# ratt-ru/pfb-imaging

Measured on AMD Instinct MI355X. Metric: Mvis/s gridded+degridded in exact Hessian applies (8192^2 grid, 1e7 vis/band), higher is better.
Workload: dtype f64

## Files before the change

### pfb-imaging_amd/csrc/gridder.hip

```cpp
#include <hip/hip_runtime.h>
#include <rocfft/rocfft.h>

#include <hipcub/hipcub.hpp>

#include <algorithm>
#include <chrono>
#include <cmath>
#include <cstdlib>
#include <string>
#include <cstring>
#include <memory>
#include <vector>

#include "common.hpp"
#include "devcg.hpp"
#include "eskernel.hpp"
#include "gridder_kernels_mp.hpp"
#include "gridder_wd_api.hpp"
#include "rowfft_api.hpp"
#include "vismap.hpp"

namespace pfbhip {

constexpr double SPEED_OF_LIGHT = 299792458.0;
// ... 568 lines not shown
        for (int q = 0; q < 3; ++q) ga.wshare[q] = wshare[q];
        return ga;
    }
    template <int W>
    size_t lds_bytes_mp() const
    {
        constexpr int D = kernel_poly_degree_c(W);
        static_assert(kernel_poly_degree_c(W) == kernel_poly_degree(W), "degree mismatch");
        return (size_t(2) * size_t(kp_max) * tile_rows(W) * tile_stride(W) + size_t(W) * (D + 1)) * sizeof(double);
    }
    template <int W>
    static constexpr size_t lds_bytes_mp_max()
    {
        constexpr int D = kernel_poly_degree_c(W);
        return (size_t(2) * KP_MAX * tile_rows(W) * tile_stride(W) + size_t(W) * (D + 1)) * sizeof(double);
    }
    template <int W, int KP>
    void launch_grid_mp_wk(const GroupArgs &ga, const double2 *sval)
    {
        allow_dynamic_lds(reinterpret_cast<const void *>(&k_grid_mp<W, KP>), int(lds_bytes_mp_max<W>()));
        hipLaunchKernelGGL((k_grid_mp<W, KP>), dim3(ga.a.nwork), dim3(MP_THREADS), lds_bytes_mp<W>(), stream, ga, sval,
                           grid_cur);
    }
    template <int W, int KP>
    size_t lds_bytes_blk() const
    {
        return (size_t(2) * KP * blk_tile_rows(W) * blk_stride(W, KP) + blk_fixed_doubles(W, blk_threads(kp_max) / 64)) * sizeof(double);
    }
    template <int W, int KP, int BC>
    void launch_grid_blk_wkb(const GroupArgs &ga, const double2 *sval)
    {
        allow_dynamic_lds(reinterpret_cast<const void *>(&k_grid_blk<W, KP, BC>), 160 * 1024);
        const size_t lds = lds_bytes_blk<W, KP>();
        PFB_REQUIRE(lds <= size_t(160) * 1024, "block scatter needs %zu bytes of LDS", lds);
        hipLaunchKernelGGL((k_grid_blk<W, KP, BC>), dim3(ga.a.nwork), dim3(blk_threads(kp_max)), lds, stream, ga, sval, grid_cur);
    }
    template <int W, int KP>
    void launch_grid_blk_wk(const GroupArgs &ga, const double2 *sval)
    {
        if constexpr (W == 14 || W == 15) {
            if (wd_bc == 2) return launch_grid_blk_wkb<W, KP, 2>(ga, sval);
        }
        launch_grid_blk_wkb<W, KP, 4>(ga, sval);
    }
    bool scatter_blk = true;
    bool scatter_rec = false, pval_ready = false, want_pval = false;
    WdArgs wd{};
    int wd_bc = 4;
    DevBuf<double> d_dtab;
    DevBuf<double2> d_cw;
    bool wd_small = false;
    int pval_per_vis() const { return info.wmode == 2 ? wd.K : kp_max; }
    bool pval_from_gather = false;
    DevBuf<VisRec> d_rec;
    bool gather_rw = false;
    DevBuf<double> d_kw;
    float wshare[3] = {1.3f / 3, 1.f / 3, 0.7f / 3};
    DevBuf<double2> d_pval;
    template <int W, int KP, int BC>
    void launch_grid_rec_wkb(const GroupArgs &ga)
    {
        allow_dynamic_lds(reinterpret_cast<const void *>(&k_grid_rec<W, KP, BC>), 160 * 1024);
        const size_t lds = lds_bytes_blk<W, KP>();
        PFB_REQUIRE(lds <= size_t(160) * 1024, "record scatter needs %zu bytes of LDS", lds);
        hipLaunchKernelGGL((k_grid_rec<W, KP, BC>), dim3(ga.a.nwork), dim3(blk_threads(kp_max)), lds, stream, ga, d_rec.p, d_pval.p,
                           grid_cur);
    }
    template <int W, int KP>
    void launch_grid_rec_wk(const GroupArgs &ga)
    {
        if constexpr (W == 14 || W == 15) {
            if (wd_bc == 2) return launch_grid_rec_wkb<W, KP, 2>(ga);
        }
        launch_grid_rec_wkb<W, KP, 4>(ga);
    }
    template <int W>
    void launch_grid_mp_w(int plane0, int kp, const double2 *sval)
    {
        GroupArgs ga = group_args(plane0, kp);
        if (ga.a.nwork == 0) return;
        if (scatter_blk) {
            const size_t grp = work_off.size() > 1 ? size_t(plane0 / kp_max) : 0;
            if (scatter_rec && !pval_ready) {
                timer.begin(5);
                if (info.wmode == 2)
                    wd_launch_plane_values(wd.K, info.nactive, d_cw.p, sval, d_pval.p, stream);
                else if (prm.do_wgridding && info.wmode == 0)
                    hipLaunchKernelGGL((k_plane_values_es<W>), dim3(ga.a.nwork), dim3(256), 0, stream, ga, sval, d_pval.p);
                else
                    hipLaunchKernelGGL((k_plane_values<W>), dim3(uint32_t(ceil_div(info.nactive, 256))), dim3(256), 0, stream, ga,
                                       info.nactive, sval, d_pval.p);
                timer.end();
            }
            for (int col = 0; col < 4; ++col) {
                ga.a.work = d_work_col.p + col_off[grp * 4 + size_t(col)];
                ga.a.nwork = uint32_t(col_cnt[grp * 4 + size_t(col)]);
                if (ga.a.nwork == 0) continue;
                timer.begin(0);
                if (info.wmode == 2) {
                    wd_launch_grid(ga, wd, d_rec.p, d_pval.p, grid_cur, stream);
                    timer.end();
                    continue;
                }
                if (scatter_rec) {
                    switch (kp) {
                        case 1: launch_grid_rec_wk<W, 1>(ga); break;
                        case 2: launch_grid_rec_wk<W, 2>(ga); break;
                        case 3: launch_grid_rec_wk<W, 3>(ga); break;
                        default: launch_grid_rec_wk<W, 4>(ga); break;
                    }
                    timer.end();
                    continue;
                }
                switch (kp) {
                    case 1: launch_grid_blk_wk<W, 1>(ga, sval); break;
                    case 2: launch_grid_blk_wk<W, 2>(ga, sval); break;
                    case 3: launch_grid_blk_wk<W, 3>(ga, sval); break;
                    default: launch_grid_blk_wk<W, 4>(ga, sval); break;
                }
                timer.end();
            }
            return;
        }
        timer.begin(0);
        switch (kp) {
            case 1: launch_grid_mp_wk<W, 1>(ga, sval); break;
            case 2: launch_grid_mp_wk<W, 2>(ga, sval); break;
            case 3: launch_grid_mp_wk<W, 3>(ga, sval); break;
            default: launch_grid_mp_wk<W, 4>(ga, sval); break;
        }
        timer.end();
    }
    template <int W, int KP>
    void launch_degrid_mp_wk(const GroupArgs &ga, double2 *sacc)
    {
        allow_dynamic_lds(reinterpret_cast<const void *>(&k_degrid_mp<W, KP>), int(lds_bytes_mp_max<W>()));
        hipLaunchKernelGGL((k_degrid_mp<W, KP>), dim3(ga.a.nwork), dim3(MP_THREADS), lds_bytes_mp<W>(), stream, ga,
                           grid_cur, sacc, want_pval ? d_swgt.p : nullptr, want_pval ? d_pval.p : nullptr);
    }
    template <int W, int KP>
    void launch_degrid_rw_wk(const GroupArgs &ga, double2 *sacc)
    {
        allow_dynamic_lds(reinterpret_cast<const void *>(&k_degrid_rw<W, KP>), 160 * 1024);
        const size_t lds = size_t(KP) * RW_LS * RW_LS * sizeof(double2);
        hipLaunchKernelGGL((k_degrid_rw<W, KP>), dim3(ga.a.nwork), dim3(MP_THREADS), lds, stream, ga, d_rec.p, d_kw.p, grid_cur,
                           sacc, want_pval ? d_swgt.p : nullptr, want_pval ? d_pval.p : nullptr);
    }
    template <int W>
    void launch_degrid_mp_w(int plane0, int kp, double2 *sacc)
    {
        GroupArgs ga = group_args(plane0, kp);
        if (ga.a.nwork == 0) return;
        if (info.wmode == 2) {
// ... 136 lines not shown
    }

    FusedGeom fgeom;
    const FusedGeom &fused_geom() const { return fgeom; }
    std::vector<FusedPlanes> plane_groups;
    DevBuf<double2> d_tau;
    FusedPlanes fused_planes(int p0, int kp) const
    {
        const size_t grp = size_t(p0 / kp_max);
        if (grp < plane_groups.size() && plane_groups[grp].kp == kp) return plane_groups[grp];
        FusedPlanes fp;
        fp.kp = kp;
        for (int k = 0; k < FUSED_MAXPLANES; ++k) fp.w[k] = k < kp ? wplanes[size_t(p0 + k)] : 0.0;
        return fp;
    }

    void finalize(const double *beam, double scale, double eta, const double *x, double *out)
    {
        const int64_t npix = int64_t(prm.nx) * prm.ny;
        timer.begin(5);
        hipLaunchKernelGGL(k_finalize_img, dim3(uint32_t(ceil_div(npix, 256))), dim3(256), 0, stream, d_accT.p, d_corr.p, beam, scale,
                           eta, x, npix, out);
        PFB_HIP(hipGetLastError());
        timer.end();
    }

    void prepare_degrid_input(const double *x, const double *beam)
    {
        const int64_t npix = int64_t(prm.nx) * prm.ny;
        timer.begin(5);
        hipLaunchKernelGGL(k_prepare_img, dim3(uint32_t(ceil_div(npix, 256))), dim3(256), 0, stream, x, d_corr.p, beam, npix,
                           d_accT.p);
        PFB_HIP(hipGetLastError());
        timer.end();
    }

    void prepare_and_degrid(const double *x, const double *beam, double2 *sacc)
    {
        if (side_clear_pending && info.nplanes == 1) side_clear();
        if (fused && info.nactive != 0 && info.nwork != 0 && fused_pad_takes_prep(rowfft_u, fgeom)) {
            FusedPrep p;
            p.x = x;
            p.corr = d_corr.p;
            p.beam = beam;
            degrid_all_planes(sacc, &p);
        } else {
            prepare_degrid_input(x, beam);
            degrid_all_planes(sacc);
        }
    }

    void degrid_all_planes(double2 *sacc, const FusedPrep *prep = nullptr)
    {
        if (!want_pval) PFB_HIP(hipMemsetAsync(sacc, 0, size_t(std::max<int64_t>(info.nactive, 1)) * sizeof(double2), stream));
        if (info.nactive == 0 || info.nwork == 0) return;
        for (int p0 = 0; p0 < info.nplanes; p0 += kp_max) {
            const int kp = int(std::min<int64_t>(kp_max, info.nplanes - p0));
            if (fused) {
                timer.begin(7);
                fused_pad_fft(rowfft_u, fused_geom(), d_occ.p, d_accT.p, prep != nullptr ? *prep : FusedPrep{},
                              fused_planes(p0, kp), prm.do_wgridding, d_gridB.p, bstride, stream);
                timer.end();
            }
            if (tfft) {
                timer.begin(2);
                rowfft_b2a(rowfft_v.pl, d_gridB.p, grid_cur, d_rowmap.p, int(occ_rows), geom.bpitch, int(prm.ny), size_t(geom.apitch),
                           fgeom.tpitch, kp, plane_stride, bstride, d_colruns.p, stream);
                timer.end();
            }
            for (int k = 0; k < kp && !tfft; ++k) {
                const int p = p0 + k;
                if (!fused) {
                    timer.begin(3);
                    hipLaunchKernelGGL(k_pad_screen_T, dim3(uint32_t(ceil_div(info.nu, 256)), uint32_t(prm.ny)),
                                       dim3(256), 0, stream, geom, fgeom, d_accT.p, prm.do_wgridding, wplanes[size_t(p)],
                                       d_gridB.p);
                    PFB_HIP(hipGetLastError());
                    timer.end();
                    fft_rows_B(true);
                }
                timer.begin(3);
                hipLaunchKernelGGL(k_b2a, tgrid(info.nu, info.nv), dim3(TP, TRANSPOSE_ROWS), 0, stream, geom, d_occ.p,
                                   d_gridB.p + (fused ? size_t(k) * bstride : 0), grid_cur + size_t(k) * plane_stride);
                PFB_HIP(hipGetLastError());
                timer.end();
                fft_rows_A(true, k);
            }
            if (side_clear_pending) side_clear();
            timer.begin(1);
            PFB_W_DISPATCH(launch_degrid_mp_w, p0, kp, sacc);
            PFB_HIP(hipGetLastError());
            timer.end();
        }
    }

    DevBuf<float> d_stage32;
    void upload_f32(const float *host, size_t n, double *dst)
    {
        d_stage32.ensure(n);
        PFB_HIP(hipMemcpyAsync(d_stage32.p, host, n * sizeof(float), hipMemcpyHostToDevice, stream));
        hipLaunchKernelGGL(k_widen_f32, dim3(uint32_t(ceil_div(int64_t(n), 256))), dim3(256), 0, stream, int64_t(n), d_stage32.p, dst);
        PFB_HIP(hipGetLastError());
    }
    void download_f32(const double *src, size_t n, float *host)
    {
        d_stage32.ensure(n);
        hipLaunchKernelGGL(k_narrow_f64, dim3(uint32_t(ceil_div(int64_t(n), 256))), dim3(256), 0, stream, int64_t(n), src, d_stage32.p);
        PFB_HIP(hipGetLastError());
        PFB_HIP(hipMemcpyAsync(host, d_stage32.p, n * sizeof(float), hipMemcpyDeviceToHost, stream));
    }
    void upload_vis_wgt_sp(const float *vis_host, const float *wgt_host)
    {
        if (vis_host) {
            d_vis.ensure(size_t(nvis));
            upload_f32(vis_host, size_t(nvis) * 2, reinterpret_cast<double *>(d_vis.p));
        }
        if (wgt_host) {
            d_wgt.ensure(size_t(nvis));
            upload_f32(wgt_host, size_t(nvis), d_wgt.p);
        }
    }
    void upload_vis_wgt(const double *vis_host, const double *wgt_host)
    {
        if (vis_host) {
            d_vis.ensure(size_t(nvis));
            PFB_HIP(hipMemcpyAsync(d_vis.p, vis_host, size_t(nvis) * sizeof(double2), hipMemcpyHostToDevice, stream));
        }
        if (wgt_host) {
            d_wgt.ensure(size_t(nvis));
            PFB_HIP(hipMemcpyAsync(d_wgt.p, wgt_host, size_t(nvis) * sizeof(double), hipMemcpyHostToDevice, stream));
        }
    }
};

namespace pfbhip {

static inline dim3 blocks1d(int64_t n, int t = 256) { return dim3(uint32_t(std::max<int64_t>(ceil_div(n, t), 1))); }

static double fft2d_seconds(int64_t nu, int64_t nv)
{
    static const struct { int64_t n; double ms; } meas[] = {
// ... 49 lines not shown
    if (!(smax >= 0.0 && smax < 1.0)) return HUGE_VAL;
    double tq[WD_MAX_K], M[WD_MAX_K][WD_MAX_K];
    wd_interp_nodes(K, smax, nshift, tq, M);
    double worst = 0.0;
    for (int iw = 0; iw <= WD_ERR_NW; ++iw) {
        const double dwv = whalf * (double(iw) / (0.5 * WD_ERR_NW) - 1.0);
        double cr[WD_MAX_K], ci[WD_MAX_K];
        for (int k = 0; k < K; ++k) {
            cr[k] = ci[k] = 0.0;
            for (int q = 0; q < K; ++q) {
                cr[k] += M[k][q] * std::cos(2.0 * pi_const * dwv * tq[q]);
                ci[k] -= M[k][q] * std::sin(2.0 * pi_const * dwv * tq[q]);
            }
        }
        for (int is = 0; is <= WD_ERR_NS; ++is) {
            const double x = double(is) / double(WD_ERR_NS), sv = x * smax;
            const double tt = -sv / (1.0 + std::sqrt(1.0 - sv)) + nshift;
            double ar = 0.0, ai = 0.0, xp = 1.0;
            for (int k = 0; k < K; ++k) {
                ar += cr[k] * xp;
                ai += ci[k] * xp;
                xp *= x;
            }
            const double e = std::hypot(ar - std::cos(2.0 * pi_const * dwv * tt), ai + std::sin(2.0 * pi_const * dwv * tt));
            if (!std::isfinite(e)) return HUGE_VAL;
            worst = std::max(worst, e);
        }
    }
    return worst;
}

static double wd_smax(const pfbhip_gridder_params &p)
{
    const double xe = double(p.nx / 2) * p.pixsize_x, ye = double(p.ny / 2) * p.pixsize_y;
    return xe * xe + ye * ye;
}

static double w_interp_budget(const pfbhip_gridder_params &p, double nmin)
{
    return 2.0 * p.epsilon / 3.0 * (p.divide_by_n ? std::max(0.25, std::min(1.0, nmin)) : 1.0);
}

enum class ScatterForce { Auto, Walk, Block, Rec, RecEs };
struct PlanSwitches {
    ScatterForce scatter = ScatterForce::Auto;
    bool wmode2 = true;
    bool wd_block4 = false;
    int wd_colours = -1;
    bool rowfft = true;
    bool fused_fft = true;
    int fused_doubled = -1;
    bool sepscreen = true;
    bool tfft = true;
};

static PlanSwitches read_plan_switches()
{
    PlanSwitches sw;
    auto first = [](const char *name) -> int {
        const char *e = std::getenv(name);
        return e == nullptr ? -1 : e[0];
    };
    if (const char *e = std::getenv("PFBHIP_SCATTER")) {
        const std::string v(e);
        if (v == "auto") sw.scatter = ScatterForce::Auto;
        else if (v == "walk") sw.scatter = ScatterForce::Walk;
        else if (v == "block") sw.scatter = ScatterForce::Block;
        else if (v == "rec") sw.scatter = ScatterForce::Rec;
        else if (v == "rec_es") sw.scatter = ScatterForce::RecEs;
        else PFB_REQUIRE(false, "PFBHIP_SCATTER=%s: expected auto, walk, block, rec or rec_es", e);
    }
    sw.wmode2 = first("PFBHIP_WMODE2") != '0';
    sw.wd_block4 = first("PFBHIP_WD_BLOCK") == '4';
    const int wc = first("PFBHIP_WD_COLOURS");
    sw.wd_colours = wc == '0' ? 0 : (wc == '1' ? 1 : -1);
    sw.rowfft = first("PFBHIP_ROWFFT") != '0';
    sw.fused_fft = first("PFBHIP_FUSED_FFT") != '0';
    const int fd = first("PFBHIP_FUSED_DOUBLED");
    sw.fused_doubled = fd < 0 ? -1 : (fd == '1' ? 1 : 0);
    sw.sepscreen = first("PFBHIP_SEPSCREEN") != '0';
    sw.tfft = first("PFBHIP_TFFT") != '0';
    return sw;
}

static void choose_kernel(pfbhip_gridder *g, const PlanSwitches &sw, double wlo, double whi, double tmax, double nmin)
{
    const auto &prm = g->prm;
    size_t nrows = 0;
    const KernelRow *tab = kernel_table(&nrows);
    const double eps1 = 0.8 / 1.25 * prm.epsilon / (prm.do_wgridding ? 3.0 : 2.0) *
                        ((prm.do_wgridding && prm.divide_by_n) ? std::max(0.25, std::min(1.0, nmin)) : 1.0);
    const double eps_w = 0.5 * w_interp_budget(prm, nmin);
    const double nvis = double(g->nvis);
    const bool wgrid = prm.do_wgridding && tmax > 0.0;
    const double pi = 3.14159265358979323846;
    double best_cost = 1e300;
    const KernelRow *best = nullptr;
    int64_t bnu = 0, bnv = 0, bnpl = 1;
    double bdw = 1.0;
    int bmode = 0, bnder = 0;
    const bool wd_allowed = sw.wmode2 && g->info.lshift == 0.0 && g->info.mshift == 0.0 &&
                            (sw.scatter == ScatterForce::Auto || sw.scatter == ScatterForce::Rec);
    const double wd_omega = 2.0 * pi * 0.5 * (whi - wlo) * tmax;
    int wd_K = 0;
    if (wgrid && wd_allowed) {
        const int K0 = poly_planes_needed(wd_omega, 2.0 * eps_w);
        for (int K = K0; K >= 2 && K <= WD_MAX_K; ++K)
            if (wd_interp_error(K, wd_smax(prm), 0.5 * (whi - wlo), g->info.nshift) <= 2.0 * eps_w) {
                wd_K = K;
                break;
            }
    }
    for (size_t i = 0; i < nrows; ++i) {
        const KernelRow &r = tab[i];
        if (prm.force_W > 0) {
            if (r.W != prm.force_W || std::fabs(r.sigma - prm.force_sigma) > 1e-9) continue;
        } else {
            if (r.sigma < prm.sigma_min - 1e-9 || r.sigma > prm.sigma_max + 1e-9 || r.eps_sup > eps1) continue;
        }
        double rounding_es = 0.0, rounding_poly = 0.0;
        int64_t cand_u[2] = {grid_size(prm.nx, r.sigma), rowfft_size_at_least(double(prm.nx) * r.sigma)};
        int64_t cand_v[2] = {grid_size(prm.ny, r.sigma), rowfft_size_at_least(double(prm.ny) * r.sigma)};
        for (int cand = 0; cand < 2; ++cand) {
            const int64_t nu = cand_u[cand], nv = cand_v[cand];
            if (nu <= 0 || nv <= 0) continue;
            if (cand == 1 && (nu == cand_u[0] && nv == cand_v[0])) continue;
            if (cand == 1 && prm.force_W <= 0 &&
                (double(nu) > prm.sigma_max * double(prm.nx) || double(nv) > prm.sigma_max * double(prm.ny)))
                continue;
            if (prm.force_W <= 0) {
                const KernelFT ft(r.W, r.beta);
                const double f0 = ft(0.0);
                double amp = (f0 / ft(0.5 * double(prm.nx) / double(nu))) * (f0 / ft(0.5 * double(prm.ny) / double(nv)));
                if (wgrid) amp = std::max(amp, amp * f0 / ft(0.5 / r.sigma));
// ... 449 lines not shown
            wd_interp_nodes(K, smax, info.nshift, wa.tq, wa.M);
            g->d_cw.alloc((size_t(info.nactive) + REC_PAD) * size_t(K));
            wa.cw = g->d_cw.p;
            wd_launch_coeffs(wa, info.nactive, g->d_pw.p, g->d_cw.p, st);
            const double worst = wd_interp_error(K, smax, info.whalf, info.nshift), bound = w_interp_budget(prm, 1.0 + nm1min);
            if (prm.verbosity > 0) fprintf(stderr, "[pfbhip] one-plane w-scheme: K = %d, interpolation error %.3g\n", K, worst);
            PFB_REQUIRE(worst <= bound, "one-plane w-scheme: interpolation error %g exceeds its share %g of epsilon %g", worst, bound,
                        prm.epsilon);
        }
        PFB_HIP(hipStreamSynchronize(st));
    }

    const int64_t npix = prm.nx * prm.ny;
    KernelFT ft(info.W, info.beta);
    std::vector<double> cfu = ft.correction_1d(prm.nx, info.nu);
    std::vector<double> cfv = (prm.ny == prm.nx && info.nv == info.nu) ? cfu : ft.correction_1d(prm.ny, info.nv);
    g->d_cfu.alloc(cfu.size());
    g->d_cfv.alloc(cfv.size());
    PFB_HIP(hipMemcpyAsync(g->d_cfu.p, cfu.data(), cfu.size() * sizeof(double), hipMemcpyHostToDevice, st));
    PFB_HIP(hipMemcpyAsync(g->d_cfv.p, cfv.data(), cfv.size() * sizeof(double), hipMemcpyHostToDevice, st));
    std::vector<double> cheb{1.0};
    double zmax = 1.0;
    const bool use_psiw = prm.do_wgridding && tmax > 0.0 && info.wmode == 0;
    if (use_psiw) {
        zmax = tmax * info.dw * (1.0 + 1e-12);
        cheb = ft.inverse_cheb(zmax);
    }
    g->d_cheb.alloc(cheb.size());
    PFB_HIP(hipMemcpyAsync(g->d_cheb.p, cheb.data(), cheb.size() * sizeof(double), hipMemcpyHostToDevice, st));
    g->d_corr.alloc(size_t(npix));
    hipLaunchKernelGGL(k_corr_image, blocks1d(npix), dim3(256), 0, st, g->geom, g->d_cfu.p, g->d_cfv.p, g->d_cheb.p,
                       int(cheb.size()), info.dw, zmax, prm.do_wgridding ? 1 : 0, use_psiw ? 1 : 0, prm.divide_by_n,
                       g->d_corr.p);
    PFB_HIP(hipGetLastError());

    lap("kernel table + correction");
    {
        RowFFTPlan probe;
        const bool own_v = sw.rowfft && rowfft_make_plan(info.nv, &probe);
        g->geom.apitch = int(info.nv) + (own_v ? 8 : 0);
    }
    g->plane_stride = size_t(info.nu) * size_t(g->geom.apitch);
    g->d_grid.alloc(g->plane_stride * size_t(g->kp_max));
    g->grid_cur = g->d_grid.p;
    {
        g->async_clear = info.nplanes <= g->kp_max && info.nactive > 0 && g->d_grid.bytes() <= (size_t(40) << 30);
        if (g->async_clear) {
            g->d_grid2.alloc(g->plane_stride * size_t(g->kp_max));
            PFB_HIP(hipStreamCreateWithFlags(&g->clear_stream, hipStreamNonBlocking));
            PFB_HIP(hipEventCreateWithFlags(&g->ev_clear, hipEventDisableTiming));
            PFB_HIP(hipEventCreateWithFlags(&g->ev_start, hipEventDisableTiming));
            PFB_HIP(hipMemsetAsync(g->d_grid2.p, 0, g->d_grid2.bytes(), st));
        }
    }
    lap("uv-plane buffers");
    g->d_img.alloc(size_t(npix));
    g->d_sval.alloc(size_t(std::max<int64_t>(info.nactive, 1)));
    g->d_sacc.alloc(size_t(std::max<int64_t>(info.nactive, 1)));

    const bool own_rows = sw.rowfft;
    const bool want_fused = sw.fused_fft;
    if (own_rows || want_fused) (void)g->rowfft_u.init(info.nu);
    const bool fuse_doubled = sw.fused_doubled >= 0 ? sw.fused_doubled == 1 : fused_doubled_stashes(g->rowfft_u);
    {
        FusedGeom &fg = g->fgeom;
        fg.nx = int(prm.nx);
        fg.ny = int(prm.ny);
        fg.nu = int(info.nu);
        fg.px = prm.pixsize_x;
        fg.py = prm.pixsize_y;
        fg.lshift = info.lshift;
        fg.mshift = info.mshift;
        fg.nshift = info.nshift;
        if (prm.do_wgridding) fused_geom_fit(fg);
        if (prm.verbosity > 0) fprintf(stderr, "[pfbhip] w-screen: n-1 polynomial with %d coefficients\n", fg.npoly);
    }
    g->fused = want_fused && g->rowfft_u.ok && (!g->rowfft_u.pl.doubled || fuse_doubled) &&
               (!prm.do_wgridding || g->fgeom.npoly > 0);
    if (!own_rows && !g->fused) g->rowfft_u.release();
    if (own_rows) (void)g->rowfft_v.init(info.nv);
    g->plane_groups.clear();
    g->d_tau.release();
    if (g->fused) {
        bool any_sep = false;
        for (int p0 = 0; p0 < info.nplanes; p0 += g->kp_max) {
            FusedPlanes fp;
            fp.kp = int(std::min<int64_t>(g->kp_max, info.nplanes - p0));
            for (int k = 0; k < FUSED_MAXPLANES; ++k) fp.w[k] = k < fp.kp ? g->wplanes[size_t(p0 + k)] : 0.0;
            if (prm.do_wgridding && !g->rowfft_u.pl.doubled) fused_planes_fit(g->fgeom, fp);
            if (fp.nsc == 0 && sw.sepscreen && prm.do_wgridding) fused_planes_fit(g->fgeom, fp, true);
            any_sep = any_sep || fp.sep != 0;
            g->plane_groups.push_back(fp);
        }
        if (any_sep) {
            g->d_tau.alloc(size_t(info.nplanes) * size_t(prm.nx));
            DevBuf<double> d_w(size_t(info.nplanes));
            PFB_HIP(hipMemcpyAsync(d_w.p, g->wplanes.data(), size_t(info.nplanes) * sizeof(double), hipMemcpyHostToDevice, st));
            fused_screen_table(g->fgeom, d_w.p, int(info.nplanes), g->d_tau.p, st);
            PFB_HIP(hipStreamSynchronize(st));
            for (size_t grp = 0; grp < g->plane_groups.size(); ++grp)
                g->plane_groups[grp].tau = g->d_tau.p + grp * size_t(g->kp_max) * size_t(prm.nx);
        }
        if (prm.verbosity > 0 && !g->plane_groups.empty()) {
            int n_sc = 0, n_sep = 0, nsc_max = 0;
            for (const FusedPlanes &fp : g->plane_groups) {
                n_sc += fp.nsc > 0 && !fp.sep;
// ... 332 lines not shown
                for (int64_t a = a0; a < std::min(a0 + 32, pu); ++a)
                    for (int64_t b = b0; b < std::min(b0 + 32, pv); ++b) out[b * pu + a] = tmp[a * int64_t(g->geom.apitch) + b];
    });
}

int pfbhip_gridder_dirty2vis(pfbhip_gridder *g, const double *dirty_host, const double *wgt_host, double *vis_host)
{
    return guarded([&] {
        PFB_REQUIRE(g && dirty_host && (vis_host || g->nvis == 0), "NULL argument");
        hipStream_t st = g->stream;
        const int64_t npix = g->prm.nx * g->prm.ny;
        PFB_HIP(hipMemcpyAsync(g->d_img.p, dirty_host, size_t(npix) * sizeof(double), hipMemcpyHostToDevice, st));
        g->upload_vis_wgt(nullptr, wgt_host);
        g->prepare_and_degrid(g->d_img.p, nullptr, g->d_sacc.p);
        if (g->nvis) {
            g->d_vis.ensure(size_t(g->nvis));
            PFB_HIP(hipMemsetAsync(g->d_vis.p, 0, size_t(g->nvis) * sizeof(double2), st));
            if (g->info.nactive)
                hipLaunchKernelGGL(k_permute_out, blocks1d(g->info.nactive), dim3(256), 0, st, g->map, g->d_src.p,
                                   g->info.nactive, g->d_sacc.p, wgt_host ? g->d_wgt.p : nullptr, int(g->shifting),
                                   g->info.lshift, g->info.mshift, g->info.nshift, g->d_vis.p);
            PFB_HIP(hipGetLastError());
            PFB_HIP(hipMemcpyAsync(vis_host, g->d_vis.p, size_t(g->nvis) * sizeof(double2), hipMemcpyDeviceToHost, st));
        }
        PFB_HIP(hipStreamSynchronize(st));
    });
}

int pfbhip_gridder_set_weights(pfbhip_gridder *g, const double *wgt_host)
{
    return guarded([&] {
        PFB_REQUIRE(g, "NULL handle");
        hipStream_t st = g->stream;
        g->upload_vis_wgt(nullptr, wgt_host);
        g->d_swgt.ensure(size_t(std::max<int64_t>(g->info.nactive, 1)));
        if (g->info.nactive)
            hipLaunchKernelGGL(k_gather_f64, blocks1d(g->info.nactive), dim3(256), 0, st, g->d_src.p, g->info.nactive,
                               wgt_host ? g->d_wgt.p : nullptr, g->d_swgt.p);
        PFB_HIP(hipGetLastError());
        PFB_HIP(hipStreamSynchronize(st));
        g->weights_bound = true;
    });
}

static void apply_op(pfbhip_gridder *g, const double *x_dev, const double *beam_dev, const double *beam_out_dev, double scale,
                     double eta, const double *addend_dev, double *out_dev)
{
    PFB_REQUIRE(g->weights_bound, "call pfbhip_gridder_set_weights before the Hessian");
    hipStream_t st = g->stream;
    const int64_t npix = g->prm.nx * g->prm.ny;
    const bool side = g->async_clear && g->info.nwork > 0;
    g->side_clear_pending = side;
    g->side_clear_done = false;
    g->want_pval = g->pval_from_gather && g->info.nwork > 0;
    struct ClearFlags {
        pfbhip_gridder *g;
        ~ClearFlags() { g->want_pval = g->pval_ready = false; }
    } clear_flags{g};
    g->prepare_and_degrid(x_dev, beam_dev, g->d_sacc.p);
    g->side_clear_pending = false;
    if (g->want_pval) {
        g->want_pval = false;
        g->pval_ready = true;
    } else {
        g->timer.begin(5);
        if (g->info.nactive)
            hipLaunchKernelGGL(k_scale_sorted, blocks1d(g->info.nactive), dim3(256), 0, st, g->info.nactive, g->d_sacc.p,
                               g->d_swgt.p, g->d_sval.p);
        PFB_HIP(hipGetLastError());
        g->timer.end();
    }
    if (g->side_clear_done) {
        PFB_HIP(hipStreamWaitEvent(st, g->ev_clear, 0));
        g->grid_cur = g->d_grid2.p;
        g->planes_cleared = true;
    }
    struct Restore {
        pfbhip_gridder *g;
        ~Restore()
        {
            g->grid_cur = g->d_grid.p;
            g->planes_cleared = false;
        }
    } restore{g};
    g->grid_and_finalize(g->d_sval.p, beam_out_dev, scale, eta, (eta != 0.0) ? addend_dev : nullptr, out_dev);
    (void)npix;
}

static void hessian_dev_impl(pfbhip_gridder *g, const double *x_dev, const double *beam_dev, double eta, double wsum,
                             double *out_dev)
{
    apply_op(g, x_dev, beam_dev, beam_dev, wsum > 0.0 ? 1.0 / wsum : 1.0, eta, eta != 0.0 ? x_dev : nullptr, out_dev);
}

int pfbhip_gridder_residual_dev(pfbhip_gridder *g, const double *model_dev, const double *beam_dev, const double *acc_dev,
                                double *out_dev)
{
    return guarded([&] {
        PFB_REQUIRE(g && model_dev && acc_dev && out_dev, "NULL argument");
        PFB_REQUIRE(model_dev != out_dev, "the residual cannot overwrite the model image");
        apply_op(g, model_dev, beam_dev, nullptr, -1.0, 1.0, acc_dev, out_dev);
        PFB_HIP(hipStreamSynchronize(g->stream));
    });
}

int pfbhip_gridder_hessian_dev(pfbhip_gridder *g, const double *x_dev, const double *beam_dev, double eta, double wsum,
                               double *out_dev)
{
    return guarded([&] {
        PFB_REQUIRE(g && x_dev && out_dev, "NULL argument");
        PFB_REQUIRE(x_dev != out_dev, "in-place Hessian is not supported");
        hessian_dev_impl(g, x_dev, beam_dev, eta, wsum, out_dev);
        PFB_HIP(hipStreamSynchronize(g->stream));
    });
// ... 210 lines not shown
```

### pfb-imaging_amd/csrc/gridder_kernels_wd.hpp

```cpp
#pragma once
#include "gridder_wd_api.hpp"

namespace pfbhip {

__host__ __device__ constexpr int wd_binom(int n, int r)
{
    return r == 0 || r == n ? 1 : (n == 2 ? 2 : (n == 3 ? 3 : 1));
}

__global__ void k_wd_coeffs(WdArgs wa, int64_t nactive, const double *__restrict__ pw, double2 *__restrict__ cw)
{
    const int64_t j = blockIdx.x * int64_t(blockDim.x) + threadIdx.x;
    if (j >= nactive + REC_PAD) return;
    double er[WD_MAX_K], ei[WD_MAX_K];
    const double dw = j < nactive ? pw[j] * wa.whalf : 0.0;
    for (int q = 0; q < wa.K; ++q) {
        double ph = dw * wa.tq[q];
        ph -= rint(ph);
        double s, c;
        sincospi(-2.0 * ph, &s, &c);
        er[q] = c;
        ei[q] = s;
    }
    for (int k = 0; k < wa.K; ++k) {
// ... 287 lines not shown
                for (int r = 0; r < NJ; ++r) asm volatile("" : "+v"(B[r])::"memory");
                kq[ld] = *reinterpret_cast<const int4 *>(rwave + roff);
#pragma unroll
                for (int p = 0; p < NJ; ++p) pq[ld][p] = *reinterpret_cast<const double2 *>(pwave + poff + p * 16);
                roff += 32u;
                poff += pbytes;
                __builtin_amdgcn_sched_barrier(0);
                double sr[NJ], si[NJ];
#pragma unroll
                for (int r = 0; r < NJ; ++r) {
                    sr[r] = pq[u][r].x * B[0];
                    si[r] = pq[u][r].y * B[0];
#pragma unroll
                    for (int m = 1; r + m < NJ; ++m) {
                        const double bm = double(wd_binom(r + m, r)) * B[m];
                        sr[r] = fma(pq[u][r + m].x, bm, sr[r]);
                        si[r] = fma(pq[u][r + m].y, bm, si[r]);
                    }
                }
#pragma unroll
                for (int k = 0; k < NR; ++k) {
                    bool on = true;
                    if (SKIP && k == 0) on = (rk.w & 0x300) != 0x300;
                    if (SKIP && k == NR - 1) on = (rk.w & 0x300) == 0x300;
                    if (on) {
#pragma unroll
                        for (int r = 0; r < NJ; ++r) {
                            are[k] = fma(A[k][r], sr[r], are[k]);
                            aim[k] = fma(A[k][r], si[r], aim[k]);
                        }
                    }
                }
                asm volatile("" ::"s"(rk.y), "s"(rk.z));
            }
        }
    }
    asm volatile("" ::"v"(warm));
    if (cur >= 0) flush(cur);
    __syncthreads();
    blk_tile_to_grid<W, 1, LS, 256>(ga, wi, lds, bu, bv, grid);
}

template <int W, int NJ, int I>
__device__ __forceinline__ void wd_steps(const char *base, const double (&ku)[NJ], double (&tr)[NJ], double (&ti)[NJ])
{
    if constexpr (I < W) {
        const double2 cell = *reinterpret_cast<const double2 *>(base + size_t(I) * RW_LS * 16);
#pragma unroll
        for (int r = 0; r < NJ; ++r) {
            fmac_row_bcast<I>(tr[r], ku[r], cell.x);
            fmac_row_bcast<I>(ti[r], ku[r], cell.y);
        }
        wd_steps<W, NJ, I + 1>(base, ku, tr, ti);
    }
}

__host__ __device__ constexpr int wd_gather_threads(int) { return 768; }

template <int W, int NJ>
__global__ void __launch_bounds__(wd_gather_threads(NJ)) k_degrid_wd(GroupArgs ga, WdArgs wa, const VisRec *__restrict__ rec,
                                                           const double2 *__restrict__ grid, double2 *__restrict__ sacc,
                                                           const double *__restrict__ swgt, double2 *__restrict__ pval_out)
{
    const PlaneArgs &a = ga.a;
    constexpr int D = kernel_poly_degree_c(W);
    constexpr int L = TILE + W - 1;
    constexpr int LL = RW_LS * RW_LS;
    extern __shared__ double lds[];
    double2 *tiles = reinterpret_cast<double2 *>(lds);

    const uint32_t item = blockIdx.x;
    if (item >= a.nwork) return;
    const WorkItem wi = a.work[item];
    const int bu = int(wi.tile / uint32_t(a.ntv)) * TILE;
    const int bv = int(wi.tile % uint32_t(a.ntv)) * TILE;
    const int NT = int(blockDim.x);
    const int wave = threadIdx.x >> 6, lane = threadIdx.x & 63;
    const int b = lane & 15, g = lane >> 4;
    const uint32_t stride = uint32_t(NT / 64) * 4;
    const uint32_t jlast = wi.end - 1;
    uint32_t j = wi.begin + wave * 4 + g;
    bool valid = j < wi.end;
    auto load_z = [&](uint32_t jj) { return *reinterpret_cast<const double2 *>(rec + min(jj, jlast)); };
    auto load_key = [&](uint32_t jj) { return rec[min(jj, jlast)].key; };
    double2 z = load_z(j);
    int key = load_key(j);
    double2 cwv[NJ];
#pragma unroll
    for (int k = 0; k < NJ; ++k) cwv[k] = wa.cw[size_t(min(j, jlast)) * NJ + k];
    {
        for (int i0 = 0; i0 < LL; i0 += 4 * NT) {
            double2 v[4];
            int idx[4];
#pragma unroll
            for (int q = 0; q < 4; ++q) {
                const int i = i0 + int(threadIdx.x) + q * NT;
                idx[q] = i;
                const int ic = min(i, LL - 1);
                const int la = ic / RW_LS, lb = ic - la * RW_LS;
                int gu = bu + la, gv = bv + lb;
                gu = gu >= a.nu ? gu % a.nu : gu;
                gv = gv >= a.nv ? gv % a.nv : gv;
                const bool in = i < LL && la < L && lb < L;
                const double2 t = grid[size_t(gu) * size_t(a.apitch) + size_t(gv)];
                v[q] = in ? t : make_double2(0.0, 0.0);
            }
// ... 58 lines not shown
#pragma unroll
            for (int r = 0; r < NJ; ++r) tr[r] = ti[r] = 0.0;
#pragma unroll
            for (int r = 0; r < NJ; ++r) asm volatile("s_nop 1" : "+v"(ku[r]));
            wd_steps<W, NJ, 0>(base, ku, tr, ti);
            double vr = 0.0, vi = 0.0;
#pragma unroll
            for (int r = 0; r < NJ; ++r) {
                double qr = cwv[r].x * B[0], qi = cwv[r].y * B[0];
#pragma unroll
                for (int m = 1; r + m < NJ; ++m) {
                    const double bm = double(wd_binom(r + m, r)) * B[m];
                    qr = fma(cwv[r + m].x, bm, qr);
                    qi = fma(cwv[r + m].y, bm, qi);
                }
                vr = fma(tr[r], qr, vr);
                vr = fma(ti[r], qi, vr);
                vi = fma(ti[r], qr, vi);
                vi = fma(-tr[r], qi, vi);
            }
            const bool lo = b < 8;
            const double keep = lo ? vr : vi, give = lo ? vi : vr;
            const double tot = half_row_sum(keep + rotn_f64<8>(give));
            const double oth = rotn_f64<8>(tot);
            if (valid) {
                if (pval_out != nullptr) {
                    if ((b & 7) < NJ) {
                        const double wj = swgt[j];
                        const double re = (lo ? tot : oth) * wj, im = (lo ? oth : tot) * wj;
                        double cr = cwv[0].x, ci = cwv[0].y;
#pragma unroll
                        for (int k = 1; k < NJ; ++k) {
                            cr = bsel == k ? cwv[k].x : cr;
                            ci = bsel == k ? cwv[k].y : ci;
                        }
                        double *o = reinterpret_cast<double *>(pval_out + size_t(j) * size_t(NJ) + size_t(bsel));
                        o[lo ? 0 : 1] = lo ? (re * cr - im * ci) : (re * ci + im * cr);
                    }
                } else if ((b & 7) == 0) {
                    double *o = reinterpret_cast<double *>(sacc + j);
                    o[lo ? 0 : 1] = tot;
                }
            }
        }
        j = jn;
        valid = nvalid;
        z = nz;
        key = nkey;
#pragma unroll
        for (int k = 0; k < NJ; ++k) cwv[k] = ncw[k];
    }
}

}
```

### pfb-imaging_amd/csrc/gridder_wd.hip

```cpp
#include "gridder_kernels_wd.hpp"

#include <algorithm>
#include <stdexcept>

#include "common.hpp"

namespace pfbhip {

static int scatter_threads_for(uint32_t nwork) { return nwork < 768u ? wd_threads() : 256; }
int wd_scatter_threads() { return wd_threads(); }
static int wd_gather_threads_rt(int NJ, uint32_t nwork) { return std::min(nwork < 768u ? 768 : 256, wd_gather_threads(NJ)); }
size_t wd_scatter_lds_bytes(int W)
{
    size_t n = 0;
    switch (W) {
#define PFB_CASE(w) case w: n = wd_lds_doubles(w, wd_scatter_threads() / 64); break;
        PFB_CASE(4) PFB_CASE(5) PFB_CASE(6) PFB_CASE(7) PFB_CASE(8) PFB_CASE(9) PFB_CASE(10) PFB_CASE(11)
        PFB_CASE(12) PFB_CASE(13) PFB_CASE(14) PFB_CASE(15) PFB_CASE(16)
#undef PFB_CASE
        default: throw std::runtime_error("unsupported kernel support");
    }
    return n * sizeof(double);
}
size_t wd_gather_lds_bytes() { return size_t(RW_LS) * RW_LS * sizeof(double2); }
// ... 35 lines not shown
    switch (wa.K) {
        case 2: grid_wk<W, 2>(ga, wa, rec, pval, grid, st); break;
        case 3: grid_wk<W, 3>(ga, wa, rec, pval, grid, st); break;
        case 4: grid_wk<W, 4>(ga, wa, rec, pval, grid, st); break;
        default: throw std::runtime_error("one-plane w-scheme: 2..4 kernel functions");
    }
}
void wd_launch_grid(const GroupArgs &ga, const WdArgs &wa, const VisRec *rec, const double2 *pval, double2 *grid, hipStream_t st)
{
    if (ga.a.nwork == 0) return;
    switch (wa.W) {
#define PFB_CASE(w) case w: grid_w<w>(ga, wa, rec, pval, grid, st); break;
        PFB_CASE(4) PFB_CASE(5) PFB_CASE(6) PFB_CASE(7) PFB_CASE(8) PFB_CASE(9) PFB_CASE(10) PFB_CASE(11)
        PFB_CASE(12) PFB_CASE(13) PFB_CASE(14) PFB_CASE(15) PFB_CASE(16)
#undef PFB_CASE
        default: throw std::runtime_error("unsupported kernel support");
    }
    PFB_HIP(hipGetLastError());
}

template <int W, int NJ>
static void degrid_wk(const GroupArgs &ga, const WdArgs &wa, const VisRec *rec, const double2 *grid, double2 *sacc,
                      const double *swgt, double2 *pval_out, hipStream_t st)
{
    allow_dynamic_lds(reinterpret_cast<const void *>(&k_degrid_wd<W, NJ>), 160 * 1024);
    hipLaunchKernelGGL((k_degrid_wd<W, NJ>), dim3(ga.a.nwork), dim3(wd_gather_threads_rt(NJ, ga.a.nwork)), wd_gather_lds_bytes(), st, ga, wa, rec, grid, sacc,
                       swgt, pval_out);
}
template <int W>
static void degrid_w(const GroupArgs &ga, const WdArgs &wa, const VisRec *rec, const double2 *grid, double2 *sacc,
                     const double *swgt, double2 *pval_out, hipStream_t st)
{
    switch (wa.K) {
        case 2: degrid_wk<W, 2>(ga, wa, rec, grid, sacc, swgt, pval_out, st); break;
        case 3: degrid_wk<W, 3>(ga, wa, rec, grid, sacc, swgt, pval_out, st); break;
        case 4: degrid_wk<W, 4>(ga, wa, rec, grid, sacc, swgt, pval_out, st); break;
        default: throw std::runtime_error("one-plane w-scheme: 2..4 kernel functions");
    }
}
void wd_launch_degrid(const GroupArgs &ga, const WdArgs &wa, const VisRec *rec, const double2 *grid, double2 *sacc,
                      const double *swgt, double2 *pval_out, hipStream_t st)
{
    if (ga.a.nwork == 0) return;
    switch (wa.W) {
#define PFB_CASE(w) case w: degrid_w<w>(ga, wa, rec, grid, sacc, swgt, pval_out, st); break;
        PFB_CASE(4) PFB_CASE(5) PFB_CASE(6) PFB_CASE(7) PFB_CASE(8) PFB_CASE(9) PFB_CASE(10) PFB_CASE(11)
        PFB_CASE(12) PFB_CASE(13) PFB_CASE(14) PFB_CASE(15) PFB_CASE(16)
#undef PFB_CASE
        default: throw std::runtime_error("unsupported kernel support");
    }
    PFB_HIP(hipGetLastError());
}

}
```

### pfb-imaging_amd/csrc/gridder_wd_api.hpp

```cpp
#pragma once
#include "gridder_kernels_mp.hpp"

namespace pfbhip {

constexpr int WD_MAX_K = 4;

struct WdArgs {
    int K;
    int W;
    int bc;
    double whalf, nshift;
    double tq[WD_MAX_K];
    double M[WD_MAX_K][WD_MAX_K];
    double su[WD_MAX_K], sv[WD_MAX_K];
    const double *dtab;
    const double2 *cw;
};

__host__ __device__ constexpr int wd_block_edge(int W, bool fine_key) { return (W == 14 || W == 15) && fine_key ? 2 : BLK_CELLS; }
int wd_scatter_threads();
size_t wd_scatter_lds_bytes(int W);
size_t wd_gather_lds_bytes();
void wd_launch_coeffs(const WdArgs &wa, int64_t nactive, const double *pw, double2 *cw, hipStream_t st);
void wd_launch_plane_values(int K, int64_t nactive, const double2 *cw, const double2 *sval, double2 *pval, hipStream_t st);
void wd_launch_grid(const GroupArgs &ga, const WdArgs &wa, const VisRec *rec, const double2 *pval, double2 *grid, hipStream_t st);
void wd_launch_degrid(const GroupArgs &ga, const WdArgs &wa, const VisRec *rec, const double2 *grid, double2 *sacc,
                      const double *swgt, double2 *pval_out, hipStream_t st);

}
```

Baseline: 3311.

## Fuse degrid, weighting and regrid into one Hessian kernel per tile

Adds a k_hess_wd kernel that, for each tile, loads the input uv-plane tile into LDS, degrids each visibility, applies the weight, and scatters the weighted value straight back into an LDS output tile. The separate degrid pass, its sacc memset, and the plane-value round trip through global memory are skipped when the fused path is enabled. This removes an intermediate write and read of per-visibility values and one kernel launch per column group. The cost is higher LDS use and register pressure, and the path only runs when one plane is used, W+BC-1 fits in 16 lanes, and the output is cleared asynchronously.

```diff
diff --git a/pfb-imaging_amd/csrc/gridder.hip b/pfb-imaging_amd/csrc/gridder.hip
--- a/pfb-imaging_amd/csrc/gridder.hip
+++ b/pfb-imaging_amd/csrc/gridder.hip
@@ -644,6 +644,7 @@
     bool wd_small = false;
     int pval_per_vis() const { return info.wmode == 2 ? wd.K : kp_max; }
     bool pval_from_gather = false;
+    bool hess_fused_ok = false, hess_fused = false;
     DevBuf<VisRec> d_rec;
     bool gather_rw = false;
     DevBuf<double> d_kw;
@@ -690,7 +691,10 @@
                 if (ga.a.nwork == 0) continue;
                 timer.begin(0);
                 if (info.wmode == 2) {
-                    wd_launch_grid(ga, wd, d_rec.p, d_pval.p, grid_cur, stream);
+                    if (hess_fused)
+                        wd_launch_hessian(ga, wd, d_rec.p, d_swgt.p, d_grid.p, grid_cur, stream);
+                    else
+                        wd_launch_grid(ga, wd, d_rec.p, d_pval.p, grid_cur, stream);
                     timer.end();
                     continue;
                 }
@@ -933,7 +937,7 @@
 
     void degrid_all_planes(double2 *sacc, const FusedPrep *prep = nullptr)
     {
-        if (!want_pval) PFB_HIP(hipMemsetAsync(sacc, 0, size_t(std::max<int64_t>(info.nactive, 1)) * sizeof(double2), stream));
+        if (!want_pval && !hess_fused) PFB_HIP(hipMemsetAsync(sacc, 0, size_t(std::max<int64_t>(info.nactive, 1)) * sizeof(double2), stream));
         if (info.nactive == 0 || info.nwork == 0) return;
         for (int p0 = 0; p0 < info.nplanes; p0 += kp_max) {
             const int kp = int(std::min<int64_t>(kp_max, info.nplanes - p0));
@@ -968,6 +972,7 @@
                 fft_rows_A(true, k);
             }
             if (side_clear_pending) side_clear();
+            if (hess_fused) continue;
             timer.begin(1);
             PFB_W_DISPATCH(launch_degrid_mp_w, p0, kp, sacc);
             PFB_HIP(hipGetLastError());
@@ -1123,6 +1128,7 @@
     int fused_doubled = -1;
     bool sepscreen = true;
     bool tfft = true;
+    bool wd_fused = true;
 };
 
 static PlanSwitches read_plan_switches()
@@ -1151,6 +1157,7 @@
     sw.fused_doubled = fd < 0 ? -1 : (fd == '1' ? 1 : 0);
     sw.sepscreen = first("PFBHIP_SEPSCREEN") != '0';
     sw.tfft = first("PFBHIP_TFFT") != '0';
+    sw.wd_fused = first("PFBHIP_WD_FUSED") != '0';
     return sw;
 }
 
@@ -1706,6 +1713,8 @@
             PFB_HIP(hipEventCreateWithFlags(&g->ev_start, hipEventDisableTiming));
             PFB_HIP(hipMemsetAsync(g->d_grid2.p, 0, g->d_grid2.bytes(), st));
         }
+        g->hess_fused_ok = sw.wd_fused && info.wmode == 2 && g->coloured && !g->wd_small && g->async_clear && info.nplanes == 1 &&
+                           wd_hessian_supported(int(info.W), g->wd.bc);
     }
     lap("uv-plane buffers");
     g->d_img.alloc(size_t(npix));
@@ -2144,14 +2153,18 @@
     const bool side = g->async_clear && g->info.nwork > 0;
     g->side_clear_pending = side;
     g->side_clear_done = false;
-    g->want_pval = g->pval_from_gather && g->info.nwork > 0;
+    g->hess_fused = g->hess_fused_ok && side;
+    g->want_pval = !g->hess_fused && g->pval_from_gather && g->info.nwork > 0;
     struct ClearFlags {
         pfbhip_gridder *g;
-        ~ClearFlags() { g->want_pval = g->pval_ready = false; }
+        ~ClearFlags() { g->want_pval = g->pval_ready = g->hess_fused = false; }
     } clear_flags{g};
     g->prepare_and_degrid(x_dev, beam_dev, g->d_sacc.p);
     g->side_clear_pending = false;
-    if (g->want_pval) {
+    if (g->hess_fused) {
+        PFB_REQUIRE(g->side_clear_done, "fused Hessian: the output plane was not cleared");
+        g->pval_ready = true;
+    } else if (g->want_pval) {
         g->want_pval = false;
         g->pval_ready = true;
     } else {
diff --git a/pfb-imaging_amd/csrc/gridder_kernels_wd.hpp b/pfb-imaging_amd/csrc/gridder_kernels_wd.hpp
--- a/pfb-imaging_amd/csrc/gridder_kernels_wd.hpp
+++ b/pfb-imaging_amd/csrc/gridder_kernels_wd.hpp
@@ -363,6 +363,20 @@
             fmac_row_bcast<I>(ti[r], ku[r], cell.y);
         }
         wd_steps<W, NJ, I + 1>(base, ku, tr, ti);
+    }
+}
+
+template <int FP, int NJ, int F>
+__device__ __forceinline__ void hess_frame_steps(const double (&ks)[NJ], const double (&pr)[NJ], const double (&pim)[NJ],
+                                                 double (&fre)[FP], double (&fim)[FP])
+{
+    if constexpr (F < FP) {
+#pragma unroll
+        for (int r = 0; r < NJ; ++r) {
+            fmac_row_bcast<F>(fre[F], ks[r], pr[r]);
+            fmac_row_bcast<F>(fim[F], ks[r], pim[r]);
+        }
+        hess_frame_steps<FP, NJ, F + 1>(ks, pr, pim, fre, fim);
     }
 }
 
@@ -527,4 +541,197 @@
     }
 }
 
-}
+__host__ __device__ constexpr bool wd_hess_fits(int W, int BC) { return W + BC - 1 <= 16; }
+__host__ __device__ constexpr size_t wd_hess_lds_bytes(int W)
+{
+    return size_t(2) * blk_tile_rows(W) * wd_stride(W) * sizeof(double) + size_t(RW_LS) * RW_LS * 16;
+}
+
+template <int W, int NJ, int BC>
+__global__ void __launch_bounds__(512) k_hess_wd(GroupArgs ga, WdArgs wa, const VisRec *__restrict__ rec, const double *__restrict__ swgt,
+                                                 const double2 *__restrict__ gin, double2 *__restrict__ gout)
+{
+    const PlaneArgs &a = ga.a;
+    constexpr int D = kernel_poly_degree_c(W);
+    constexpr int L = TILE + W - 1;
+    constexpr int LS = wd_stride(W);
+    constexpr int LL = blk_tile_rows(W) * LS;
+    constexpr int LLI = RW_LS * RW_LS;
+    constexpr int FP = W + BC - 1;
+    static_assert(BC == 2 || BC == 4, "block edge: 2 or 4 cells");
+    static_assert(wd_hess_fits(W, BC), "frame wider than a 16-lane row");
+    extern __shared__ double lds[];
+    double2 *tin = reinterpret_cast<double2 *>(lds + 2 * LL);
+
+    const uint32_t item = blockIdx.x;
+    if (item >= a.nwork) return;
+    const WorkItem wi = a.work[item];
+    const int bu = int(wi.tile / uint32_t(a.ntv)) * TILE;
+    const int bv = int(wi.tile % uint32_t(a.ntv)) * TILE;
+    const int NT = int(blockDim.x);
+    const int wave = threadIdx.x >> 6, lane = threadIdx.x & 63;
+    const int b = lane & 15, g = lane >> 4, rowl = lane & ~15;
+    const uint32_t n = wi.end - wi.begin, NS = uint32_t(NT / 64) * 4, sidx = uint32_t(wave) * 4 + uint32_t(g);
+    uint32_t j = wi.begin + uint32_t((uint64_t(n) * sidx) / NS);
+    const uint32_t jend = wi.begin + uint32_t((uint64_t(n) * (sidx + 1)) / NS);
+    const uint32_t niter = (n + NS - 1) / NS;
+    const uint32_t jlast = wi.end - 1;
+    auto load_z = [&](uint32_t jj) { return *reinterpret_cast<const double2 *>(rec + min(jj, jlast)); };
+    auto load_key = [&](uint32_t jj) { return rec[min(jj, jlast)].key; };
+    double2 z = load_z(j);
+    int key = load_key(j);
+    double wv = j < jend ? swgt[min(j, jlast)] : 0.0;
+    double2 cwv[NJ];
+#pragma unroll
+    for (int k = 0; k < NJ; ++k) cwv[k] = wa.cw[size_t(min(j, jlast)) * NJ + k];
+
+    for (int i = threadIdx.x; i < 2 * LL; i += NT) lds[i] = 0.0;
+    for (int i0 = 0; i0 < LLI; i0 += 4 * NT) {
+        double2 v[4];
+        int idx[4];
+#pragma unroll
+        for (int q = 0; q < 4; ++q) {
+            const int i = i0 + int(threadIdx.x) + q * NT;
+            idx[q] = i;
+            const int ic = min(i, LLI - 1);
+            const int la = ic / RW_LS, lb = ic - la * RW_LS;
+            int gu = bu + la, gv = bv + lb;
+            gu = gu >= a.nu ? gu % a.nu : gu;
+            gv = gv >= a.nv ? gv % a.nv : gv;
+            const bool in = i < LLI && la < L && lb < L;
+            const double2 t = gin[size_t(gu) * size_t(a.apitch) + size_t(gv)];
+            v[q] = in ? t : make_double2(0.0, 0.0);
+        }
+#pragma unroll
+        for (int q = 0; q < 4; ++q)
+            if (idx[q] < LLI) tin[idx[q]] = v[q];
+    }
+    double c0[D + 1], c1[D - 1], c2[NJ > 2 ? D - 3 : 1], c3[NJ > 3 ? D - 5 : 1];
+#pragma unroll
+    for (int q = 0; q <= D; ++q) c0[q] = b < W ? wa.dtab[(size_t(0) * W + b) * (D + 1) + q] : 0.0;
+#pragma unroll
+    for (int q = 0; q <= D - 2; ++q) c1[q] = b < W ? wa.dtab[(size_t(1) * W + b) * (D + 1) + q] : 0.0;
+    if constexpr (NJ > 2) {
+#pragma unroll
+        for (int q = 0; q <= D - 4; ++q) c2[q] = b < W ? wa.dtab[(size_t(2) * W + b) * (D + 1) + q] : 0.0;
+    }
+    if constexpr (NJ > 3) {
+#pragma unroll
+        for (int q = 0; q <= D - 6; ++q) c3[q] = b < W ? wa.dtab[(size_t(3) * W + b) * (D + 1) + q] : 0.0;
+    }
+    auto evens = [](const auto &c, auto deg, double zz) {
+        constexpr int DG = decltype(deg)::value;
+        const double z2 = zz * zz;
+        double e = c[DG], o = c[DG - 1];
+#pragma unroll
+        for (int k = DG - 2; k >= 0; k -= 2) {
+            e = fma(e, z2, c[k]);
+            if (k >= 1) o = fma(o, z2, c[k - 1]);
+        }
+        return fma(o, zz, e);
+    };
+    auto kernel_values = [&](double zz, const double *scale, double (&out)[NJ]) {
+        out[0] = evens(c0, std::integral_constant<int, D>{}, zz);
+        out[1] = evens(c1, std::integral_constant<int, D - 2>{}, zz) * scale[1];
+        if constexpr (NJ > 2) out[2] = evens(c2, std::integral_constant<int, D - 4>{}, zz) * scale[2];
+        if constexpr (NJ > 3) out[3] = evens(c3, std::integral_constant<int, D - 6>{}, zz) * scale[3];
+    };
+
+    double fre[FP], fim[FP];
+#pragma unroll
+    for (int f = 0; f < FP; ++f) fre[f] = fim[f] = 0.0;
+    int cur = -1;
+    auto flush = [&]() {
+        const int r0 = cur >> 8, cc = cur & 255;
+        double *o = lds + r0 * LS + cc + b;
+        if (b < FP) {
+#pragma unroll
+            for (int f = 0; f < FP; ++f) {
+                unsafeAtomicAdd(o + f * LS, fre[f]);
+                unsafeAtomicAdd(o + LL + f * LS, fim[f]);
+            }
+        }
+#pragma unroll
+        for (int f = 0; f < FP; ++f) fre[f] = fim[f] = 0.0;
+    };
+    __syncthreads();
+
+    const char *tbase = reinterpret_cast<const char *>(tin);
+    for (uint32_t it = 0; it < niter; ++it) {
+        const bool valid = j < jend;
+        const uint32_t jn = j + 1;
+        const double2 nz = load_z(jn);
+        const int nkey = load_key(jn);
+        const double nwv = jn < jend ? swgt[min(jn, jlast)] : 0.0;
+        double2 ncw[NJ];
+#pragma unroll
+        for (int k = 0; k < NJ; ++k) ncw[k] = wa.cw[size_t(min(jn, jlast)) * NJ + k];
+        {
+            double ku[NJ], kvb[NJ];
+            kernel_values(z.x, wa.su, ku);
+            kernel_values(z.y, wa.sv, kvb);
+            const int lu = key >> 8, lv = key & 255;
+            const int du = lu & (BC - 1), dv = lv & (BC - 1);
+            const int c0c = lv - dv;
+            double B[NJ], ks[NJ];
+#pragma unroll
+            for (int r = 0; r < NJ; ++r) B[r] = __shfl(kvb[r], rowl + ((b - dv) & 15));
+#pragma unroll
+            for (int r = 0; r < NJ; ++r) ks[r] = __shfl(ku[r], rowl + ((b - du) & 15));
+            const char *base = tbase + (lu * RW_LS + c0c + b) * 16;
+            double tr[NJ], ti[NJ];
+#pragma unroll
+            for (int r = 0; r < NJ; ++r) tr[r] = ti[r] = 0.0;
+#pragma unroll
+            for (int r = 0; r < NJ; ++r) asm volatile("s_nop 1" : "+v"(ku[r]));
+            wd_steps<W, NJ, 0>(base, ku, tr, ti);
+            double sr[NJ], si[NJ];
+            double vr = 0.0, vi = 0.0;
+#pragma unroll
+            for (int r = 0; r < NJ; ++r) {
+                sr[r] = cwv[r].x * B[0];
+                si[r] = cwv[r].y * B[0];
+#pragma unroll
+                for (int m = 1; r + m < NJ; ++m) {
+                    const double bm = double(wd_binom(r + m, r)) * B[m];
+                    sr[r] = fma(cwv[r + m].x, bm, sr[r]);
+                    si[r] = fma(cwv[r + m].y, bm, si[r]);
+                }
+                vr = fma(tr[r], sr[r], vr);
+                vr = fma(ti[r], si[r], vr);
+                vi = fma(ti[r], sr[r], vi);
+                vi = fma(-tr[r], si[r], vi);
+            }
+            const bool lo = b < 8;
+            const double keep = lo ? vr : vi, give = lo ? vi : vr;
+            const double tot = half_row_sum(keep + rotn_f64<8>(give));
+            const double oth = rotn_f64<8>(tot);
+            const double wr = (lo ? tot : oth) * wv, wi_ = (lo ? oth : tot) * wv;
+            double pr[NJ], pim[NJ];
+#pragma unroll
+            for (int r = 0; r < NJ; ++r) {
+                pr[r] = wr * sr[r] - wi_ * si[r];
+                pim[r] = wr * si[r] + wi_ * sr[r];
+            }
+            const int blk = valid ? (((lu - du) << 8) | c0c) : cur;
+            if (blk != cur) {
+                if (cur >= 0) flush();
+                cur = blk;
+            }
+#pragma unroll
+            for (int r = 0; r < NJ; ++r) asm volatile("s_nop 1" : "+v"(ks[r]));
+            hess_frame_steps<FP, NJ, 0>(ks, pr, pim, fre, fim);
+        }
+        j = jn;
+        z = nz;
+        key = nkey;
+        wv = nwv;
+#pragma unroll
+        for (int k = 0; k < NJ; ++k) cwv[k] = ncw[k];
+    }
+    if (cur >= 0) flush();
+    __syncthreads();
+    blk_tile_to_grid<W, 1, LS, 256>(ga, wi, lds, bu, bv, gout);
+}
+
+}
diff --git a/pfb-imaging_amd/csrc/gridder_wd.hip b/pfb-imaging_amd/csrc/gridder_wd.hip
--- a/pfb-imaging_amd/csrc/gridder_wd.hip
+++ b/pfb-imaging_amd/csrc/gridder_wd.hip
@@ -111,4 +111,40 @@
     PFB_HIP(hipGetLastError());
 }
 
+template <int W, int NJ, int BC>
+static void hess_wkb(const GroupArgs &ga, const WdArgs &wa, const VisRec *rec, const double *swgt, const double2 *gin, double2 *gout,
+                     hipStream_t st)
+{
+    allow_dynamic_lds(reinterpret_cast<const void *>(&k_hess_wd<W, NJ, BC>), 160 * 1024);
+    hipLaunchKernelGGL((k_hess_wd<W, NJ, BC>), dim3(ga.a.nwork), dim3(256), wd_hess_lds_bytes(W), st, ga, wa, rec, swgt, gin, gout);
 }
+template <int W, int BC>
+static void hess_wb(const GroupArgs &ga, const WdArgs &wa, const VisRec *rec, const double *swgt, const double2 *gin, double2 *gout,
+                    hipStream_t st)
+{
+    switch (wa.K) {
+        case 2: hess_wkb<W, 2, BC>(ga, wa, rec, swgt, gin, gout, st); break;
+        case 3: hess_wkb<W, 3, BC>(ga, wa, rec, swgt, gin, gout, st); break;
+        case 4: hess_wkb<W, 4, BC>(ga, wa, rec, swgt, gin, gout, st); break;
+        default: throw std::runtime_error("one-plane w-scheme: 2..4 kernel functions");
+    }
+}
+bool wd_hessian_supported(int W, int bc) { return W >= 4 && W <= 16 && (bc == 2 || bc == 4) && wd_hess_fits(W, bc) && (bc == 4 || W >= 14); }
+void wd_launch_hessian(const GroupArgs &ga, const WdArgs &wa, const VisRec *rec, const double *swgt, const double2 *gin, double2 *gout,
+                       hipStream_t st)
+{
+    if (ga.a.nwork == 0) return;
+    if (!wd_hessian_supported(wa.W, wa.bc)) throw std::runtime_error("fused Hessian: W + block edge - 1 must be <= 16");
+    switch (wa.W) {
+#define PFB_CASE(w) case w: hess_wb<w, 4>(ga, wa, rec, swgt, gin, gout, st); break;
+        PFB_CASE(4) PFB_CASE(5) PFB_CASE(6) PFB_CASE(7) PFB_CASE(8) PFB_CASE(9) PFB_CASE(10) PFB_CASE(11)
+        PFB_CASE(12) PFB_CASE(13)
+#undef PFB_CASE
+        case 14: hess_wb<14, 2>(ga, wa, rec, swgt, gin, gout, st); break;
+        case 15: hess_wb<15, 2>(ga, wa, rec, swgt, gin, gout, st); break;
+        default: throw std::runtime_error("unsupported kernel support");
+    }
+    PFB_HIP(hipGetLastError());
+}
+
+}
diff --git a/pfb-imaging_amd/csrc/gridder_wd_api.hpp b/pfb-imaging_amd/csrc/gridder_wd_api.hpp
--- a/pfb-imaging_amd/csrc/gridder_wd_api.hpp
+++ b/pfb-imaging_amd/csrc/gridder_wd_api.hpp
@@ -26,5 +26,8 @@
 void wd_launch_grid(const GroupArgs &ga, const WdArgs &wa, const VisRec *rec, const double2 *pval, double2 *grid, hipStream_t st);
 void wd_launch_degrid(const GroupArgs &ga, const WdArgs &wa, const VisRec *rec, const double2 *grid, double2 *sacc,
                       const double *swgt, double2 *pval_out, hipStream_t st);
+bool wd_hessian_supported(int W, int bc);
+void wd_launch_hessian(const GroupArgs &ga, const WdArgs &wa, const VisRec *rec, const double *swgt, const double2 *gin, double2 *gout,
+                       hipStream_t st);
 
 }
```

After: 3777, median of 6. 14.1% higher.
